# ChaoqinRobotics/LINS---LiDAR-inertial-SLAM

Measured on AMD Instinct MI355X. Metric: ESKF iterations/sec (16x1800 VLP-16, ~2k feat), higher is better.
Workload: dtype f64 state / f32 points

## Files before the change

lins---lidar-inertial-slam_amd/csrc/ieskf_lds_impl.h:

```cpp

#include <hip/hip_runtime.h>

#include "ieskf_binned.h"
#include "ieskf_device.h"
#include "ieskf_grid.h"
#include "icp_math.h"
#include "icp_wave.h"
#include "ieskf_rowsum.h"

#ifndef LINS_PERSIST
#define LINS_PERSIST 0
#endif
#ifndef LINS_PRIO_SHIFT
#define LINS_PRIO_SHIFT 0
#endif
#ifndef LINS_PRIO_LEVEL
#define LINS_PRIO_LEVEL 3
#endif
#ifndef LINS_WALK_CACHE
#define LINS_WALK_CACHE 1
#endif
#ifndef LINS_SPREAD_S
#define LINS_SPREAD_S 5
#define LINS_SPREAD_C 3
#endif

namespace lins {
namespace LINS_LDS_NS {

struct OutRec {
  double residual_norm, update_norm;
  int iters, converged, diverged, m_surf, m_corner, pad[3];
};

struct KernelArgs {
  DevParams prm;
  const ScanDesc* descs;
  const int* order;
  const GridTables* tabs;
  const double* state_in;
  const double* cov_in;
  const double* lin_in;
  double* state_out;
  double* a6_out;
  double* cov_out;
  OutRec* out;
  lins_pose_record* poses;
  double* sums_out;
  int* counts_out;
  long long* prof_buf;
  double* relay_hdr;
  int* relay_lane;
  int* queue;
  int* relay_err;
  unsigned* walk_cache;
  int run_gen;
  int iter_arg, scan_id_base, relay_n, relay_at, relay_cuts, relay_gen;
  int relay_cap;
  int relay_items;
  int relay_spins;
};
typedef const KernelArgs __attribute__((address_space(4))) * ColdArgs;
__device__ __forceinline__ ColdArgs cold_args() {
  auto p = __builtin_amdgcn_kernarg_segment_ptr();
  asm volatile("" : "+s"(p));
  return (ColdArgs)p;
}

constexpr int kMaxLWaves = LINS_LDS_WAVES;
#ifndef LINS_LDS_BATCH_BLOCK
#define LINS_LDS_BATCH_BLOCK 512
#endif
constexpr int kBatchBlock = LINS_LDS_BATCH_BLOCK;
constexpr int kNpCap = LINS_LDS_CAP;
constexpr int kNpMax = LINS_LDS_NMAX;
constexpr bool kHybrid = kNpMax > kNpCap;
constexpr int kScanBatch = LINS_LDS_SCANBATCH;
static_assert(kNpMax >= kNpCap && kNpMax <= kGridNpMax, "positions are u16, indices u16; the index kernel's cap");

typedef unsigned v4u __attribute__((ext_vector_type(4)));
struct LdsStore {
  float4 pt[kNpCap];
  GridTables gt;
  double P[324];
  double trig[kSincCosTab];
  IterConst ic;
  double filt[19];
  double sums[28];
  double partial[kMaxLWaves * 28 > kIcpWorkspace ? kMaxLWaves * 28 : kIcpWorkspace];
  double aug[3][42];
  double res_prev, res_last, upd_norm;
  int scan_tmp[kMaxLWaves + 4];
  int m_surf, m_corner, iter, conv, div, pad;
  long long prof_acc[16];
#ifdef LINS_PROF_TAIL
  long long prof_tail[2];
#endif
#ifdef LINS_PROF2
  int prof2[64];
  int prof3[32];
#endif
  int dbg[4];
};
static_assert(sizeof(LdsStore) <= LINS_LDS_BYTES, "LDS budget of one workgroup");

__shared__ LdsStore g_lds;

struct LCloud {
  const unsigned short* cell_end;
  const int* ring_start;
  const float2* el_ang;
  int naz, stride, base, n;
  const float4* gs;
  int n_lds;
};

__device__ __forceinline__ void pt_xyz(const LdsStore& L, const LCloud& c, int p, float& x, float& y, float& z) {
  if (!kHybrid || p < c.n_lds) {
    const float4 v = L.pt[p];
    x = v.x, y = v.y, z = v.z;
  } else {
    const float4 g = c.gs[p];
    x = g.x, y = g.y, z = g.z;
  }
}
__device__ __forceinline__ int pt_idx(const LdsStore& L, const LCloud& c, int p) {
  if (!kHybrid || p < c.n_lds) return __float_as_int(L.pt[p].w);
  return __float_as_int(c.gs[p].w);
}
__device__ __forceinline__ float pt_sqdist(const LdsStore& L, const LCloud& c, int p, float sx, float sy, float sz) {
  float x, y, z;
  pt_xyz(L, c, p, x, y, z);
  return sqdist3(x, y, z, sx, sy, sz);
}

struct QueryPolar {
  float rho, qn3, el, inv_unused;
  int a0_surf_or_corner;
};

struct Best {
  unsigned long long k;
  int pos, ring;
  unsigned long long k2;
  int pos2, ring2;
  float omin;
  __device__ __forceinline__ float d() const { return __uint_as_float((unsigned)(k >> 32)); }
  __device__ __forceinline__ int key() const { return (int)(unsigned)k; }
};
__device__ __forceinline__ Best best_init(float thr) {
  return Best{(unsigned long long)__float_as_uint(thr) << 32, -1, -1, 0x7F800000FFFFFFFFull, -1, -1, INFINITY};
}
__device__ __forceinline__ unsigned long long pack_key(float d, int key) {
  return ((unsigned long long)__float_as_uint(d) << 32) | (unsigned)key;
}
__device__ __forceinline__ void insert_key(Best& b, unsigned long long k, int pos, int ring) {
  if (k < b.k) {
    if (b.pos2 >= 0) b.omin = fminf(b.omin, __uint_as_float((unsigned)(b.k2 >> 32)));
    b.k2 = b.k, b.pos2 = b.pos, b.ring2 = b.ring;
    b.k = k, b.pos = pos, b.ring = ring;
  } else if (k > b.k) {
    if (k < b.k2) {
      if (b.pos2 >= 0) b.omin = fminf(b.omin, __uint_as_float((unsigned)(b.k2 >> 32)));
      b.k2 = k, b.pos2 = pos, b.ring2 = ring;
    } else if (k > b.k2) {
      b.omin = fminf(b.omin, __uint_as_float((unsigned)(k >> 32)));
    }
  }
}
__device__ __forceinline__ void consider(Best& b, float d, int key, int pos, int ring) {
  insert_key(b, pack_key(d, key), pos, ring);
}
__device__ __forceinline__ void consider_scan(Best& b, bool ok, float d, int key, int pos, int ring) {
  const bool cand = ok && d <= __uint_as_float((unsigned)(b.k2 >> 32));
  b.omin = (ok && !cand) ? fminf(b.omin, d) : b.omin;
  if (cand) insert_key(b, pack_key(d, key), pos, ring);
}
__device__ __forceinline__ void merge_from_lane(Best& b, int src_lane) {
  unsigned lo = __shfl((unsigned)b.k, src_lane), hi = __shfl((unsigned)(b.k >> 32), src_lane);
  unsigned lo2 = __shfl((unsigned)b.k2, src_lane), hi2 = __shfl((unsigned)(b.k2 >> 32), src_lane);
  int pos = __shfl(b.pos, src_lane), ring = __shfl(b.ring, src_lane);
  int pos2 = __shfl(b.pos2, src_lane), ring2 = __shfl(b.ring2, src_lane);
  float om = __shfl(b.omin, src_lane);
  b.omin = fminf(b.omin, om);
  if (pos >= 0) insert_key(b, ((unsigned long long)hi << 32) | lo, pos, ring);
  if (pos2 >= 0) insert_key(b, ((unsigned long long)hi2 << 32) | lo2, pos2, ring2);
}

template <int LANES>
__device__ __forceinline__ void merge_query_lanes(Best& b, int lane_base, int role, int ln) {
  if (LANES == 3) {
    merge_from_lane(b, lane_base + (role + 1) % 3);
    merge_from_lane(b, lane_base + (role + 2) % 3);
  } else if (LANES != 1) {
    const int n = LANES ? LANES : ln;
#pragma unroll 1
    for (int m = 1; m < n; m <<= 1) merge_from_lane(b, lane_base + (role ^ m));
  }
}

__device__ __forceinline__ float bound_sqrtf(float x) { return __builtin_amdgcn_sqrtf(x); }

__device__ __forceinline__ float bound_divf(float x, float y) { return x * __frcp_rn(y) * (1.f + 3e-7f); }

__device__ __forceinline__ float cert_lb(const Best& b, float thr, float margin) {
  return fminf(bound_sqrtf(b.omin), bound_sqrtf(b.pos >= 0 ? b.d() : thr) + margin);
}
__device__ __forceinline__ bool certified(float d_now, float lb, float drift) {
  return bound_sqrtf(d_now) * (1.f + 4e-6f) + 2e-6f < (lb - drift * (1.f + 4e-6f)) * (1.f - 4e-6f);
}


#ifndef LINS_GLOB_BATCH
#define LINS_GLOB_BATCH 1
#endif
constexpr int kGlobBatch = LINS_GLOB_BATCH;
struct Spans {
  int s0, e0, s1, e1, spans;
  __device__ __forceinline__ int count() const { return (e0 - s0) + (e1 - s1); }
};
__device__ __forceinline__ Spans spans_of(const LCloud& c, int r, int lo, int hi) {
  int s0 = 0, e0 = 0, s1 = 0, e1 = 0, spans = 1;
  if (lo <= hi) {
    const int naz = c.naz, row = r * naz;
    int len = hi - lo;
    if (len >= naz - 1) lo = 0, len = naz - 1;
    lo &= naz - 1;
    hi = lo + len;
    const int c0 = row + lo, c1 = row + (hi < naz ? hi : naz - 1);
    s0 = c0 ? (int)c.cell_end[c0 - 1] : c.base;
    e0 = (int)c.cell_end[c1];
    if (hi >= naz) {
      spans = 2;
      s1 = row ? (int)c.cell_end[row - 1] : c.base;
      e1 = (int)c.cell_end[row + hi - naz];
    }
  }
  return Spans{s0, e0, s1, e1, spans};
}
template <class F>
__device__ __forceinline__ void scan_spans(const LdsStore& L, const LCloud& c, const Spans& w, F f) {
#pragma unroll 1
  for (int k = 0; k < w.spans; ++k) {
    const int s = k ? w.s1 : w.s0, e = k ? w.e1 : w.e0;
    const int el = kHybrid ? (e < c.n_lds ? e : c.n_lds) : e;
#pragma unroll 1
// ... 324 lines not shown
  NnOut r{bb.pos, bb.ring, bb.pos2, bb.ring2, cert_lb(bb, thr, margin)};
  if (ln > 1) {
    const int src = (cm.rank * ln) & 63;
    r.pos = __shfl(r.pos, src), r.ring = __shfl(r.ring, src);
    r.pos2 = __shfl(r.pos2, src), r.ring2 = __shfl(r.ring2, src), r.lb = __shfl(r.lb, src);
  }
  return r;
}
__device__ __forceinline__ WalkOut coop_walk(const LdsStore& L, const LCloud& c, bool is_surf, int nq, const CoopMap& cm, int coop_cap,
                                             bool need_walk, int lane, float sx, float sy, float sz, const QueryPolar& qp, int j1, int rho1,
                                             int w2, int w3, bool nn_changed, float thr, float margin, bool skip) {
  const int ln = coop_lanes(cm.n, coop_cap);
  const int wrole = lane & (ln - 1), wbase = lane - wrole, item = lane / ln;
  bool valid = need_walk;
  float isx = sx, isy = sy, isz = sz;
  QueryPolar iq = qp;
  int i_j1 = j1, i_rho1 = rho1, i_w2 = w2, i_w3 = w3, i_chk = nn_changed;
  if (ln > 1) {
    valid = item < cm.n;
    const int owner = __shfl(cm.owner_map, valid ? item : 0);
    isx = __shfl(sx, owner), isy = __shfl(sy, owner), isz = __shfl(sz, owner);
    iq.rho = __shfl(qp.rho, owner), iq.qn3 = __shfl(qp.qn3, owner), iq.el = __shfl(qp.el, owner);
    iq.a0_surf_or_corner = __shfl(qp.a0_surf_or_corner, owner);
    i_j1 = __shfl(j1, owner), i_rho1 = __shfl(rho1, owner);
    i_w2 = __shfl(w2, owner), i_w3 = __shfl(w3, owner), i_chk = __shfl((int)nn_changed, owner);
  }
  Best c2 = best_init(thr), c3 = c2;
  if (valid && !skip)
    walk_lds<0>(L, c, is_surf, nq, thr, i_j1, i_rho1, isx, isy, isz, iq, margin, ln, wrole, wbase, i_w2, i_w3, i_chk != 0, c2, c3);
  WalkOut r{c2.pos, c2.pos2, c3.pos, c3.pos2, cert_lb(c2, thr, margin), cert_lb(c3, thr, margin)};
  if (ln > 1) {
    const int src = (cm.rank * ln) & 63;
    r.r2 = __shfl(r.r2, src), r.r2b = __shfl(r.r2b, src), r.r3 = __shfl(r.r3, src), r.r3b = __shfl(r.r3b, src);
    r.lb2 = __shfl(r.lb2, src), r.lb3 = __shfl(r.lb3, src);
  }
  return r;
}
constexpr int kRelayLanes = 512;
constexpr int kRelayRegionInts = 4 * kRelayLanes * 4;
constexpr int kRelayLaneInts = kRelayRegionInts;
#ifdef LINS_LDS_LEAN
#include "ieskf_lds_lean.h"
constexpr bool kLeanBuild = true;
#else
constexpr bool kLeanBuild = false;
#endif
__device__ __forceinline__ LCloud make_cloud(const LdsStore& L, bool is_surf, const float4* gs, int n_corner_t, int n_surf_t, int n_lds) {
  return is_surf ? LCloud{L.gt.cell_end + kCellsCorner, L.gt.ring_start[0], &L.gt.el_ang[0][0], kAzSurf, 1, n_corner_t, n_surf_t, gs, n_lds}
                 : LCloud{L.gt.cell_end, L.gt.ring_start[1], &L.gt.el_ang[1][0], kAzCorner, kAzSurf / kAzCorner, 0, n_corner_t, gs, n_lds};
}
template <int BLOCK>
#ifndef LINS_GRID_INLINE
#define LINS_GRID_INLINE 1
#endif
#if LINS_GRID_INLINE
__device__ __forceinline__
#else
__device__ __noinline__
#endif
    void
    load_lds_grid(const GridTables* __restrict__ tab, const float4* __restrict__ gs, int n_lds, int tid) {
  LdsStore& L = g_lds;
  constexpr int kTabPer = (kGridTableWords + BLOCK - 1) / BLOCK, kPtPer = (kNpCap + BLOCK - 1) / BLOCK;
  constexpr int kChunk = kPtPer < 12 ? kPtPer : 12;
  const uint4* src = reinterpret_cast<const uint4*>(tab);
  uint4* dst = reinterpret_cast<uint4*>(&L.gt);
  uint4 tw[kTabPer];
#pragma unroll
  for (int u = 0; u < kTabPer; ++u) tw[u] = src[min(tid + u * BLOCK, kGridTableWords - 1)];
  if (n_lds > 0) {
#pragma unroll
    for (int k0 = 0; k0 < kPtPer; k0 += kChunk) {
      float4 pbuf[kChunk];
#pragma unroll
      for (int u = 0; u < kChunk; ++u) pbuf[u] = gs[min(tid + (k0 + u) * BLOCK, n_lds - 1)];
#pragma unroll
      for (int u = 0; u < kChunk; ++u) L.pt[min(tid + (k0 + u) * BLOCK, n_lds - 1)] = pbuf[u];
    }
  }
#pragma unroll
  for (int u = 0; u < kTabPer; ++u) dst[min(tid + u * BLOCK, kGridTableWords - 1)] = tw[u];
  __syncthreads();
}

#include "ieskf_lds_tail.h"

__device__ __forceinline__ void relay_st(int* p, int v) { __hip_atomic_store(p, v, __ATOMIC_RELAXED, __HIP_MEMORY_SCOPE_AGENT); }
__device__ __forceinline__ int relay_ld(const int* p) { return __hip_atomic_load(p, __ATOMIC_RELAXED, __HIP_MEMORY_SCOPE_AGENT); }
__device__ __forceinline__ void relay_st(double* p, double v) {
  __hip_atomic_store(reinterpret_cast<long long*>(p), __double_as_longlong(v), __ATOMIC_RELAXED, __HIP_MEMORY_SCOPE_AGENT);
}
__device__ __forceinline__ double relay_ld(const double* p) {
  return __longlong_as_double(__hip_atomic_load(reinterpret_cast<const long long*>(p), __ATOMIC_RELAXED, __HIP_MEMORY_SCOPE_AGENT));
}
__device__ __forceinline__ int relay_add(int* p, int v) { return __hip_atomic_fetch_add(p, v, __ATOMIC_RELAXED, __HIP_MEMORY_SCOPE_AGENT); }

#ifndef LINS_RELAY_RELEASE
#define LINS_RELAY_RELEASE 1
#endif
__device__ __forceinline__ void relay_raise(int* p, int v) {
  __hip_atomic_fetch_max(p, v, LINS_RELAY_RELEASE ? __ATOMIC_RELEASE : __ATOMIC_RELAXED, __HIP_MEMORY_SCOPE_AGENT);
}
__device__ __forceinline__ int relay_ld_acq(const int* p) {
  return __hip_atomic_load(p, LINS_RELAY_RELEASE ? __ATOMIC_ACQUIRE : __ATOMIC_RELAXED, __HIP_MEMORY_SCOPE_AGENT);
}

constexpr int kQHead = 0, kQExited = 32, kQFlags = 64;


template <int BLOCK, int LANES, bool PASS_ONLY, bool PROF, bool ICP, bool KNOBS>
__device__ __forceinline__ bool ieskf_lds_update(const KernelArgs ka, const float4* __restrict__ arena, const float4* __restrict__ sorted,
                                                 int4* __restrict__ idx_store, lins_corr* __restrict__ dump, const int scan, const int part) {
  const bool cont = part > 0;
  const DevParams prm = ka.prm;
  const int relay_n = ka.relay_n, relay_at = ka.relay_at;
  const int pad = KNOBS ? prm.pad : 0;
  constexpr bool prof = PROF;
  constexpr int kLBlock = BLOCK, kQPerWave = 64 / LANES, kQPerRound = (BLOCK / 64) * kQPerWave;
  static_assert(BLOCK >= 256 && BLOCK / 64 <= kMaxLWaves, "block shape");
  LdsStore& L = g_lds;
  if (prof && threadIdx.x < 16) g_lds.prof_acc[threadIdx.x] = 0;
#ifdef LINS_PROF2
  if (prof && threadIdx.x < 64) g_lds.prof2[threadIdx.x] = 0;
  if (prof && threadIdx.x < 32) g_lds.prof3[threadIdx.x] = 0;
#define PROF2_ADD(ph, dt)                                                                   \
  do {                                                                                      \
    if (prof && lane == 0 && iter >= LINS_PROF2 && wave < 8) g_lds.prof2[wave * 8 + (ph)] += (int)(dt); \
  } while (0)
#else
#define PROF2_ADD(ph, dt) \
  do {                    \
    (void)sizeof(dt);     \
  } while (0)
#endif
  const long long t_begin = prof ? clock64() : 0, t_wall_begin = prof ? wall_clock64() : 0;
  const int tid = threadIdx.x, lane = tid & 63, wave = __builtin_amdgcn_readfirstlane(tid >> 6);
  constexpr bool kLean = kLeanBuild && LANES == 1 && !PASS_ONLY && !ICP;
  constexpr bool kRelay = kLean && BLOCK == kBatchBlock;
  const ScanDesc sd = ka.descs[scan];
  const int total = sd.n_surf_q + sd.n_corner_q;
  const float4* const gs = sorted + sd.off_surf_t;
  const int n_all_t = sd.n_surf_t + sd.n_corner_t, n_lds = n_all_t < kNpCap ? n_all_t : kNpCap;

  for (int k = tid; k < 324; k += kLBlock) L.P[k] = (PASS_ONLY || ICP) ? 0.0 : ka.cov_in[(size_t)scan * 324 + k];
  if (tid < 19) {
    double v = ka.state_in[(size_t)scan * 19 + tid];
    L.filt[tid] = v;
    L.ic.lin[tid] = PASS_ONLY ? ka.lin_in[(size_t)scan * 19 + tid] : v;
  }
  if (tid < 28) L.sums[tid] = 0;
  if (tid == 64) lins_sinc_cos_table(L.trig);
  if (tid == 0) {
    L.res_prev = 1e6, L.res_last = 0, L.upd_norm = 0;
    L.iter = PASS_ONLY ? ka.iter_arg : 0, L.conv = 0, L.div = 0, L.m_surf = 0, L.m_corner = 0;
    L.dbg[0] = L.dbg[1] = L.dbg[2] = L.dbg[3] = 0;
  }
  __syncthreads();
  if (tid < 64 && !(kRelay && cont)) {
    IterConst ic;
    double filt[19];
    for (int k = 0; k < 19; ++k) ic.lin[k] = L.ic.lin[k], filt[k] = L.filt[k];
    make_iter_const_tail(filt, ic);
    if (tid == 0) {
      L.ic.phi = ic.phi, L.ic.Rt = ic.Rt, L.ic.Gt = ic.Gt;
      for (int k = 0; k < 18; ++k) L.ic.d[k] = ic.d[k];
    }
  }
  load_lds_grid<BLOCK>(ka.tabs + scan, gs, n_lds, tid);
  if (prof && tid == 0) L.prof_acc[0] = clock64() - t_begin;

  const LCloud cs{L.gt.cell_end + kCellsCorner, L.gt.ring_start[0], &L.gt.el_ang[0][0], kAzSurf, 1, sd.n_corner_t, sd.n_surf_t,
                  gs, n_lds};
  const LCloud cc{L.gt.cell_end, L.gt.ring_start[1], &L.gt.el_ang[1][0], kAzCorner, kAzSurf / kAzCorner, 0, sd.n_corner_t,
                  gs, n_lds};
  const int role = lane % LANES, lane_base = lane - role, q_in_wave = lane / LANES;
  const bool lane_used = lane < kQPerWave * LANES;
  struct WrLay {
    int n_wr, k;
    bool kind_s;
    int slot;
    bool active;
  };
  constexpr int kWaves = BLOCK / 64, kSpreadSurf = LINS_SPREAD_S > 0 && BLOCK == kBatchBlock ? LINS_SPREAD_S : (kWaves * 5 + 4) / 8;
  constexpr int kWs = kSpreadSurf;
  constexpr int kWc = LINS_SPREAD_C > 0 && BLOCK == kBatchBlock ? LINS_SPREAD_C : kWaves - kWs;
#ifndef LINS_SPREAD_WS
#define LINS_SPREAD_WS 30, 24, 20, 14, 12
#endif
#ifndef LINS_SPREAD_WC
#define LINS_SPREAD_WC 1, 1, 1
#endif
  constexpr int kWtS[] = {LINS_SPREAD_WS, 1, 1, 1, 1, 1, 1, 1, 1, 1, 1, 1, 1, 1, 1, 1, 1}, kWtC[] = {LINS_SPREAD_WC, 1, 1, 1, 1, 1, 1, 1, 1, 1, 1, 1, 1, 1, 1, 1, 1};
  constexpr int kSpreadMax = 16;
  static_assert(LANES != 1 || kWaves <= kSpreadMax + 1, "spread layout: weights for every wave");
  constexpr bool kWeighted = BLOCK == kBatchBlock && LINS_SPREAD_S > 0;
  auto share_start = [&](const int* wt, int nw, int n, int j) {
    int tot = 0, cum = 0;
#pragma unroll
    for (int k = 0; k < kSpreadMax; ++k) tot += k < nw ? (kWeighted ? wt[k] : 1) : 0, cum += k < j ? (kWeighted ? wt[k] : 1) : 0;
    return j >= nw ? n : (n * cum) / tot;
  };
  bool fits = kWs < kWaves;
#pragma unroll
  for (int k = 0; k < kSpreadMax; ++k) {
    if (k < kWs) fits = fits && share_start(kWtS, kWs, sd.n_surf_q, k + 1) - share_start(kWtS, kWs, sd.n_surf_q, k) <= 64;
    if (k < kWc) fits = fits && share_start(kWtC, kWc, sd.n_corner_q, k + 1) - share_start(kWtC, kWc, sd.n_corner_q, k) <= 64;
  }
  const bool spread_ok = fits;
  auto wr_layout = [&](int rnd) {
    WrLay y;
    y.k = rnd * kWaves + wave;
    if (spread_ok) {
#ifdef LINS_SPREAD_ROLES
      constexpr int kRole[] = {LINS_SPREAD_ROLES, 8, 9, 10, 11, 12, 13, 14, 15, 16};
      const int role_k = (kWeighted && y.k < kWs + kWc && y.k < 8) ? kRole[y.k] : y.k;
#else
      const int role_k = y.k;
#endif
      y.n_wr = kWs + kWc, y.kind_s = role_k < kWs;
      const int j = y.kind_s ? role_k : role_k - kWs, nw = y.kind_s ? kWs : kWc, n = y.kind_s ? sd.n_surf_q : sd.n_corner_q;
      const int q0 = share_start(y.kind_s ? kWtS : kWtC, nw, n, j), q1 = share_start(y.kind_s ? kWtS : kWtC, nw, n, j + 1);
      y.slot = (y.kind_s ? 0 : sd.n_surf_q) + q0 + lane, y.active = y.k < y.n_wr && lane < q1 - q0;
    } else {
      const int nws = (sd.n_surf_q + 63) >> 6;
      y.n_wr = nws + ((sd.n_corner_q + 63) >> 6), y.kind_s = y.k < nws;
      const int q0 = y.kind_s ? y.k * 64 : (y.k - nws) * 64;
      const int left = (y.kind_s ? sd.n_surf_q : sd.n_corner_q) - q0;
      y.slot = (y.kind_s ? 0 : sd.n_surf_q) + q0 + lane, y.active = y.k < y.n_wr && lane < (left < 64 ? left : 64);
    }
    return y;
  };

  int a1 = -1, b1c = -1, ra1 = -1, rb1 = -1;
  int a2 = -1, b2c = -1, a3 = -1, b3c = -1;
  int sel1 = -1;
  float lb1 = 0.f, lb2 = 0.f, lb3 = 0.f, certA[3] = {0.f, 0.f, 0.f}, certB[3] = {0.f, 0.f, 0.f};
  bool have_cert = false;
  bool searched = false;
  constexpr int kRelayHdr = 64;
  static_assert(sizeof(IterConst) == 58 * sizeof(double), "relay header layout");
  static_assert(kGridNpMax < 32768, "grid positions travel as signed 16-bit words");
  if (kRelay && cont) {
    const double* h = ka.relay_hdr + (size_t)scan * kRelayHdr;
    if (tid < 58) reinterpret_cast<double*>(&L.ic)[tid] = relay_ld(h + tid);
    if (tid == 64) L.res_prev = relay_ld(h + 58), L.res_last = relay_ld(h + 59), L.upd_norm = relay_ld(h + 60);
    if (tid == 65) {
      const int* hi = reinterpret_cast<const int*>(h + 61);
      L.iter = relay_ld(hi), L.dbg[0] = relay_ld(hi + 1), L.dbg[1] = relay_ld(hi + 2), L.dbg[2] = relay_ld(hi + 3), L.dbg[3] = relay_ld(hi + 4);
    }
    searched = true;
    __syncthreads();
  }
  bool relay_out = false;
  const int cut_at = (kRelay && relay_n > 0) ? relay_next_cut(L.iter, relay_at, ka.relay_cuts) : 0x7FFFFFFF;
#ifdef LINS_PROF2
  int dbg_nn = 0, dbg_walk = 0, dbg_walk_mask = 0, dbg_slot = -1;
#endif

  for (;;) {
    const int iter = L.iter;
    if (!PASS_ONLY && (iter >= prm.num_iter || L.conv || L.div)) break;
    if (kRelay && iter >= cut_at) {
      relay_out = true;
      break;
    }
    __syncthreads();
    if (tid == 0) L.m_surf = 0, L.m_corner = 0;

    const bool do_search = PASS_ONLY || (iter % prm.icp_freq) == 0;
    double acc = 0;
    int ms = 0, mc = 0;
    long long t0 = prof ? clock64() : 0, t1 = t0, t2 = t0, t3 = t0;
    int surf_waves = (sd.n_surf_q + kQPerWave - 1) / kQPerWave;
    const bool aligned = surf_waves * kQPerWave + sd.n_corner_q <= kQPerRound;
    const int n_wr = LANES == 1 ? wr_layout(0).n_wr : 0;
    const int span = LANES == 1 ? ((n_wr + kWaves - 1) / kWaves) * kQPerRound
                                : (aligned ? surf_waves * kQPerWave + sd.n_corner_q : total);
    int4 held = make_int4(0, 0, 0, -1);
    int part_k = wave;
    for (int base = 0; base < span; base += kQPerRound) {
      const int vslot = base + wave * kQPerWave + q_in_wave;
      int slot = vslot;
      bool active = lane_used && vslot < span;
      bool kind_s = true;
      int wr_k = 0;
      if (LANES == 1) {
        const WrLay y = wr_layout(base / kQPerRound);
        wr_k = y.k, kind_s = y.kind_s, slot = y.slot, active = y.active;
        if (base == 0) part_k = wave;
      } else if (aligned) {
        if (wave < surf_waves)
          active = active && vslot < sd.n_surf_q;
        else
          slot = vslot - surf_waves * kQPerWave + sd.n_surf_q;
      }
      double row[7] = {0, 0, 0, 0, 0, 0, 0};
      if (span > kQPerRound) {
        a1 = b1c = ra1 = rb1 = a2 = b2c = a3 = b3c = sel1 = -1, have_cert = false;
        lb1 = lb2 = lb3 = 0.f;
      }
      if constexpr (kLean) {
#ifdef LINS_LDS_LEAN
#include "ieskf_lds_lean_body.inc"
#endif
      } else if constexpr (LANES == 1) {
        const bool is_surf = kind_s;
        const int qi = is_surf ? slot : slot - sd.n_surf_q;
        const LCloud& c = is_surf ? cs : cc;
        const float thr = prm.nearest_f;
        const bool single_round = span <= kQPerRound;
        const bool warm_iter = single_round && searched;
        const float margin = warm_iter ? prm.margin_warm : prm.margin_cold;
        const bool verify = (pad & 8) != 0;
        const int coop_cap = warm_iter ? kCoopMaxLanes : LINS_COOP_COLD;
        const unsigned long long kNone = ~0ull;
        float4 q = make_float4(0.f, 0.f, 0.f, 0.f);
        V3 phi = L.ic.phi;
        QueryOut o;
        o.accepted = 0;
        o.c[0] = o.c[1] = o.c[2] = o.c[3] = 0.f;
        o.sel[0] = o.sel[1] = o.sel[2] = 0.f;
        QueryPolar qp = {0.f, 0.f, 0.f, 0.f, 0};
        bool qp_ready = false;
        int p1 = -1, p2 = -1, p3 = -1;
        long long s0 = prof ? clock64() : 0, s1 = s0, s2 = s0;
        if (active) {
          if (pad & 0x400000)
            q = make_float4(1.f + lane, 2.f, 0.5f, 3.25f);
          else
            q = arena[(is_surf ? sd.off_surf_q : sd.off_corner_q) + qi];
          V3 t{L.ic.lin[0], L.ic.lin[1], L.ic.lin[2]};
          if (pad & 0x100000)
            o.sel[0] = q.x, o.sel[1] = q.y, o.sel[2] = q.z;
          else
            transform_to_start(prm, phi, t, q, o.sel[0], o.sel[1], o.sel[2], g_lds.trig);
        }
        if (prof) {
          s1 = clock64();
#ifndef LINS_PROF_WAVES
          if (tid == 0) L.prof_acc[6] += s1 - s0;
#endif
          PROF2_ADD(0, s1 - s0);
        }
        auto dist_to = [&](int pos) { return pt_sqdist(L, c, pos, o.sel[0], o.sel[1], o.sel[2]); };
        auto drift_from = [&](const float* cp) {
          float ex = o.sel[0] - cp[0], ey = o.sel[1] - cp[1], ez = o.sel[2] - cp[2];
          return bound_sqrtf(ex * ex + ey * ey + ez * ez);
        };
        if (do_search) {
          if (!single_round) a1 = b1c = a2 = b2c = a3 = b3c = sel1 = -1;
          bool need_nn = false, said = false, flip = false;
          int pred = -1;
          if (active && (pad & 0x80000) && warm_iter) {
            pred = a1, said = true;
          } else if (active) {
            const float da = a1 >= 0 ? dist_to(a1) : INFINITY, db = b1c >= 0 ? dist_to(b1c) : INFINITY;
            bool ok = warm_iter && !(pad & 16) && certified(fminf(fminf(da, db), thr), lb1, drift_from(certA));
            const unsigned long long ka = da < thr ? pack_key(da, pt_idx(L, c, a1)) : kNone;
            const unsigned long long kb = db < thr ? pack_key(db, pt_idx(L, c, b1c)) : kNone;
            flip = kb < ka;
            pred = (flip ? kb : ka) == kNone ? -1 : (flip ? b1c : a1);
            said = ok;
            if (verify) ok = false;
            need_nn = !ok;
          }
          {
            const CoopMap cm = coop_map(need_nn, lane);
#ifdef LINS_PROF2
            if (prof && lane == 0 && iter >= LINS_PROF2 && cm.n) g_lds.prof3[wave * 4 + 0] += 1, g_lds.prof3[wave * 4 + 2] += cm.n;
#endif
            int r_pos = -1, r_ring = -1, r_pos2 = -1, r_ring2 = -1;
            float r_lb = 0.f;
            if (cm.n) {
              if (!(pad & 0x200000)) qp = polar_of(o.sel[0], o.sel[1], o.sel[2], c.naz), qp_ready = true;
              const NnOut r = coop_nn(L, c, cm, coop_cap, need_nn, lane, o.sel[0], o.sel[1], o.sel[2], qp, ring_of(q.w), a1, ra1, thr, margin, (pad & 2) != 0);
              r_pos = r.pos, r_ring = r.ring, r_pos2 = r.pos2, r_ring2 = r.ring2, r_lb = r.lb;
            }
            if (need_nn) {
              p1 = r_pos;
              if (said && p1 != pred) atomicAdd(&L.dbg[0], 1);
              a1 = r_pos, ra1 = r_ring, b1c = r_pos2, rb1 = r_ring2;
              lb1 = r_lb;
              certA[0] = o.sel[0], certA[1] = o.sel[1], certA[2] = o.sel[2];
            } else if (active) {
              p1 = pred;
              if (flip) {
                const int tp = a1, tr = ra1;
                a1 = b1c, ra1 = rb1, b1c = tp, rb1 = tr;
              }
              atomicAdd(&L.dbg[1], 1);
            }
          }
          const bool nn_changed = p1 != sel1;
          bool set_ok = !nn_changed;
          if (LINS_WALK_CACHE && !PASS_ONLY && warm_iter && nn_changed && active && ka.walk_cache && !(pad & 0x800000)) {
            const auto rs = __builtin_amdgcn_make_buffer_rsrc(ka.walk_cache + (size_t)sd.slot_base * 8, 0, total * 32, 0x00020000);
            const unsigned gen16 = (unsigned)ka.run_gen << 16;
            const v4u e0 = __builtin_amdgcn_raw_buffer_load_b128(rs, slot * 32, 0, 16);
            const v4u e1 = __builtin_amdgcn_raw_buffer_load_b128(rs, slot * 32 + 16, 0, 16);
            if (sel1 >= 0) {
              __builtin_amdgcn_raw_buffer_store_b128(v4u{gen16 | (unsigned)sel1, ((unsigned)a2 & 0xFFFFu) | ((unsigned)b2c << 16),
                                                         ((unsigned)a3 & 0xFFFFu) | ((unsigned)b3c << 16), __float_as_uint(lb2)},
                                                     rs, slot * 32, 0, 16);
              __builtin_amdgcn_raw_buffer_store_b128(v4u{__float_as_uint(lb3), __float_as_uint(certB[0]), __float_as_uint(certB[1]),
                                                         __float_as_uint(certB[2])},
                                                     rs, slot * 32 + 16, 0, 16);
            }
            if (p1 >= 0 && e0.x == (gen16 | (unsigned)p1)) {
              a2 = (int)(short)(e0.y & 0xFFFFu), b2c = (int)e0.y >> 16, a3 = (int)(short)(e0.z & 0xFFFFu), b3c = (int)e0.z >> 16;
              lb2 = __uint_as_float(e0.w), lb3 = __uint_as_float(e1.x);
              certB[0] = __uint_as_float(e1.y), certB[1] = __uint_as_float(e1.z), certB[2] = __uint_as_float(e1.w);
              set_ok = true;
            }
          }
          if (active) sel1 = p1;
          if (prof) {
            s2 = clock64();
#ifndef LINS_PROF_WAVES
            if (tid == 0) L.prof_acc[7] += s2 - s1;
#endif
// ... 169 lines not shown
            const bool said = ok;
            if (verify) ok = false;
            if (!ok) {
              if ((pad & 32) && __ffsll(__ballot(1)) - 1 == lane) atomicAdd(&L.dbg[3], 1 + (iter >= 3 ? 1000 : 0));
              Best bb = best_init(thr);
              if (!(pad & 2))
                bb = nn_lds<LANES>(L, c, o.sel[0], o.sel[1], o.sel[2], qp, thr, margin, ring_of(q.w), LANES, role, lane_base,
                                   a1, ra1);
              p1 = bb.pos;
              if (said && p1 != pred && role == 0) atomicAdd(&L.dbg[0], 1);
              a1 = bb.pos, ra1 = bb.ring, b1c = bb.pos2, rb1 = bb.ring2;
              lb1 = cert_lb(bb, thr, margin);
              certA[0] = o.sel[0], certA[1] = o.sel[1], certA[2] = o.sel[2];
            } else {
              p1 = pred;
              if (flip) {
                const int tp = a1, tr = ra1;
                a1 = b1c, ra1 = rb1, b1c = tp, rb1 = tr;
              }
              if (role == 0) atomicAdd(&L.dbg[1], 1);
            }
          }
          const bool nn_changed = p1 != sel1;
          sel1 = p1;
          if (prof) {
            s2 = clock64();
#ifndef LINS_PROF_WAVES
            if (tid == 0) L.prof_acc[7] += s2 - s1;
#endif
          }
          if (p1 >= 0) {
            const int j1 = pt_idx(L, c, p1), rho1 = ra1;
            bool need_walk = nn_changed || !have_cert;
            int pred2 = -1, pred3 = -1;
            bool flip2 = false, flip3 = false, said23 = false;
            if (!need_walk) {
              const WalkCtx w = make_walk_ctx(c, is_surf ? sd.n_surf_q : sd.n_corner_q, j1, rho1);
              const float dB = drift_from(certB);
              auto judge = [&](int pa, int pb, float lb, int& pred, bool& flip) {
                const float da = pa >= 0 ? dist_to(pa) : INFINITY, db = pb >= 0 ? dist_to(pb) : INFINITY;
                int rka = 0, rkb = 0;
                if (pa >= 0) walk_rank(w, pt_idx(L, c, pa), rka);
                if (pb >= 0) walk_rank(w, pt_idx(L, c, pb), rkb);
                const unsigned long long ka = da < thr ? pack_key(da, rka) : kNone;
                const unsigned long long kb = db < thr ? pack_key(db, rkb) : kNone;
                flip = kb < ka;
                pred = (flip ? kb : ka) == kNone ? -1 : (flip ? pb : pa);
                return certified(fminf(fminf(da, db), thr), lb, dB);
              };
              bool ok23 = judge(a2, b2c, lb2, pred2, flip2);
              if (is_surf) ok23 = judge(a3, b3c, lb3, pred3, flip3) && ok23;
              said23 = ok23;
              need_walk = !ok23 || verify;
            }
            if (need_walk) {
              if ((pad & 32) && __ffsll(__ballot(1)) - 1 == lane) atomicAdd(&L.dbg[0], 1 + (iter >= 3 ? 1000 : 0));
              Best c2 = best_init(thr), c3 = c2;
              if (!(pad & 1))
                walk_lds<LANES>(L, c, is_surf, is_surf ? sd.n_surf_q : sd.n_corner_q, thr, j1, rho1, o.sel[0], o.sel[1],
                                o.sel[2], qp, margin, LANES, role, lane_base, a2, a3, nn_changed, c2, c3);
              if (said23 && (c2.pos != pred2 || (is_surf && c3.pos != pred3)) && role == 0) atomicAdd(&L.dbg[0], 1);
              p2 = c2.pos, p3 = c3.pos;
              a2 = c2.pos, b2c = c2.pos2, a3 = c3.pos, b3c = c3.pos2;
              lb2 = cert_lb(c2, thr, margin), lb3 = cert_lb(c3, thr, margin);
              certB[0] = o.sel[0], certB[1] = o.sel[1], certB[2] = o.sel[2];
            } else {
              p2 = pred2, p3 = pred3;
              if (flip2) {
                const int tp = a2;
                a2 = b2c, b2c = tp;
              }
              if (flip3) {
                const int tp = a3;
                a3 = b3c, b3c = tp;
              }
              if (role == 0) atomicAdd(&L.dbg[2], 1);
            }
          }
          have_cert = single_round;
#ifndef LINS_PROF_WAVES
          if (prof && tid == 0) L.prof_acc[8] += clock64() - s2;
#endif
          if (prm.icp_freq > 1 && role == 0) {
            if (ICP && !is_surf)
              held = make_int4(p1, p2, p3, sd.slot_base + slot);
            else
              idx_store[sd.slot_base + slot] = make_int4(p1, p2, p3, 0);
          }
        } else {
          int4 s = idx_store[sd.slot_base + slot];
          p1 = s.x, p2 = s.y, p3 = s.z;
        }
        long long s3 = prof ? clock64() : 0;
        asm volatile("" ::: "memory");
        if (role == 0) {
          auto pt4 = [&](int pos) {
            float4 v = make_float4(0.f, 0.f, 0.f, 0.f);
            pt_xyz(L, c, pos, v.x, v.y, v.z);
            return v;
          };
          if (is_surf) {
            if (p2 >= 0 && p3 >= 0) surf_row(prm, iter, o.sel[0], o.sel[1], o.sel[2], pt4(p1), pt4(p2), pt4(p3), o);
          } else if (p2 >= 0) {
            corner_row(prm, iter, o.sel[0], o.sel[1], o.sel[2], pt4(p1), pt4(p2), o);
          }
          if (o.accepted) {
            if (ICP) {
              const IcpRow ir = icp_row_dev(prm.inv_period, phi.x, phi.y, phi.z, q.x, q.y, q.z, q.w, o.c[0], o.c[1], o.c[2], o.c[3]);
#pragma unroll
              for (int k = 0; k < 7; ++k) row[k] = ir.v[k];
            } else {
              V3 cv{(double)o.c[0], (double)o.c[1], (double)o.c[2]};
              V3 u = cross(V3{(double)q.x, (double)q.y, (double)q.z}, mvec(L.ic.Rt, cv));
              V3 a = mvec(L.ic.Gt, u);
              row[0] = cv.x, row[1] = cv.y, row[2] = cv.z, row[3] = a.x, row[4] = a.y, row[5] = a.z;
              row[6] = prm.lidar_scale * (double)o.c[3];
            }
            if (is_surf)
              ++ms;
            else
              ++mc;
          }
          if (PASS_ONLY && dump) {
            lins_corr r;
            r.ind1 = p1 >= 0 ? pt_idx(L, c, p1) : -1;
            r.ind2 = p2 >= 0 ? pt_idx(L, c, p2) : -1;
            r.ind3 = (is_surf && p3 >= 0) ? pt_idx(L, c, p3) : -1;
            r.accepted = o.accepted;
            for (int k = 0; k < 4; ++k) r.coeff[k] = o.c[k];
            r.sel[0] = o.sel[0], r.sel[1] = o.sel[1], r.sel[2] = o.sel[2], r.sel[3] = q.w;
            dump[sd.slot_base + slot] = r;
          }
        }
#ifndef LINS_PROF_WAVES
        if (prof && tid == 0) L.prof_acc[9] += clock64() - s3;
#endif
      }
      if (prof) t1 = clock64();
#ifdef LINS_PROF_WAVES
      if (prof && lane == 0 && iter >= LINS_PROF_WAVES) L.prof_acc[6 + wave] += t1 - t0;
#endif
      if (!(pad & 0x40000)) {
        const long long r0 = prof ? clock64() : 0;
        const double red = wave_reduce_rows(row, lane);
        if (prof) PROF2_ADD(4, clock64() - r0);
        acc += red;
      }
    }
    if (do_search) searched = true;
    {
      const int sidx28 = reduce_sum_index(lane);
      if (sidx28 >= 0) L.partial[part_k * 28 + sidx28] = acc;
    }
    if (ms) atomicAdd(&L.m_surf, ms);
    if (mc) atomicAdd(&L.m_corner, mc);
    const long long b0 = prof ? clock64() : 0;
    __syncthreads();
    const long long b1 = prof ? clock64() : 0;
    PROF2_ADD(5, b1 - b0);
    if (tid < 28) {
      double sacc = 0;
#pragma unroll
      for (int g = 0; g < BLOCK / 64; ++g) sacc += L.partial[g * 28 + tid];
      L.sums[tid] = sacc;
    }
    __syncthreads();
    if (prof) t2 = clock64();
    PROF2_ADD(6, t2 - b1);
    if (PASS_ONLY && (pad & 4) && !L.conv) {
      __syncthreads();
      if (tid == 0) L.conv = 1;
      continue;
    }
    if (PASS_ONLY) {
      if (ka.sums_out && tid < 28) ka.sums_out[(size_t)scan * 28 + tid] = L.sums[tid];
      if (ka.counts_out && tid == 0) ka.counts_out[scan * 2] = L.m_surf, ka.counts_out[scan * 2 + 1] = L.m_corner;
      return true;
    }

    if (ICP && held.w >= 0 && L.m_surf >= 10) idx_store[held.w] = make_int4(held.x, held.y, held.z, 0);
    if (ICP) {
      if (tid < 64) icp_solve_and_update(tid, iter);
      __syncthreads();
    } else
      t3 = solve_and_update(prm.r2, prm.fixed_iters, pad, tid, iter, prof);
    if (prof) {
      long long t4 = clock64();
      PROF2_ADD(7, t4 - t2);
      if (tid == 0) {
        L.prof_acc[1] += t1 - t0, L.prof_acc[2] += t2 - t1, L.prof_acc[3] += t3 - t2, L.prof_acc[4] += t4 - t3;
#ifndef LINS_PROF_WAVES
        if (iter < 3) L.prof_acc[10 + iter] = t4 - t0;
#endif
      }
    }
  }
  const ColdArgs kp = cold_args();
#define KP(f) kp->f
#ifdef LINS_PROF2
  if (prof && dbg_slot >= 0) idx_store[dbg_slot] = make_int4(dbg_nn, dbg_walk, dbg_walk_mask, ra1 | (a3 >= 0 ? 0x100 : 0));
#endif
  if (prof && tid == 0) {
    long long* prof_out = KP(prof_buf);
    L.prof_acc[5] = clock64() - t_begin;
#ifndef LINS_PROF_WAVES
    L.prof_acc[13] = (long long)(unsigned)__builtin_amdgcn_s_getreg((4 << 0) | (0 << 6) | (31 << 11)) |
                     ((long long)(unsigned)__builtin_amdgcn_s_getreg((20 << 0) | (0 << 6) | (31 << 11)) << 32);
#endif
    L.prof_acc[14] = t_wall_begin, L.prof_acc[15] = wall_clock64();
    for (int k = 0; k < 16; ++k) prof_out[(size_t)scan * 16 + k] = L.prof_acc[k];
#ifdef LINS_PROF2
    int* ext = reinterpret_cast<int*>(prof_out + (size_t)gridDim.x * 16) + (size_t)scan * 64;
    for (int k = 0; k < 64; ++k) ext[k] = (k & 7) == 4 ? (L.prof3[(k >> 3) * 4 + 1] | (L.prof3[(k >> 3) * 4 + 3] << 12) | (L.prof3[(k >> 3) * 4 + 0] << 20) | (L.prof3[(k >> 3) * 4 + 2] << 26)) : L.prof2[k];
#endif
  }

  if (kRelay && relay_out) {
    double* h = KP(relay_hdr) + (size_t)scan * kRelayHdr;
    if (tid < 58) relay_st(h + tid, reinterpret_cast<const double*>(&L.ic)[tid]);
    if (tid == 64) relay_st(h + 58, L.res_prev), relay_st(h + 59, L.res_last), relay_st(h + 60, L.upd_norm);
    if (tid == 65) {
      int* hi = reinterpret_cast<int*>(h + 61);
      relay_st(hi, L.iter), relay_st(hi + 1, L.dbg[0]), relay_st(hi + 2, L.dbg[1]), relay_st(hi + 3, L.dbg[2]), relay_st(hi + 4, L.dbg[3]);
    }
    __builtin_amdgcn_fence(__ATOMIC_RELEASE, "workgroup");
    asm volatile("s_waitcnt vmcnt(0)" ::: "memory");
    __syncthreads();
    if (tid == 0) relay_raise(KP(queue) + kQFlags + scan, KP(relay_gen) * 16 + part + 1);
    return false;
  }
  if (kRelay && relay_n > 0 && tid == 0)
    relay_raise(KP(queue) + kQFlags + scan, KP(relay_gen) * 16 + 15);

  const int div = L.div;
  if (ICP) {
    if (tid < 19) KP(state_out)[(size_t)scan * 19 + tid] = (tid < 3 || (tid >= 6 && tid < 10)) ? L.ic.lin[tid] : L.filt[tid];
  } else {
    if (tid < 19) KP(state_out)[(size_t)scan * 19 + tid] = div ? L.filt[tid] : L.ic.lin[tid];
    if (KP(a6_out) && tid < 21) KP(a6_out)[(size_t)scan * 21 + tid] = L.sums[tid];
  }
  if (tid == 0) {
    OutRec r;
    r.residual_norm = L.res_last, r.update_norm = L.upd_norm;
    r.iters = L.iter, r.converged = L.conv, r.diverged = div;
    r.m_surf = L.m_surf, r.m_corner = L.m_corner;
    r.pad[0] = L.dbg[0], r.pad[1] = (pad & 32) ? L.dbg[3] : L.dbg[1], r.pad[2] = L.dbg[2];
    KP(out)[scan] = r;
  }
  if (KP(poses) && tid < 32) {
    lins_pose_record* pr = KP(poses) + scan;
    const double* st = div ? L.filt : L.ic.lin;
    if (tid < 19) pr->state[tid] = st[tid];
    if (tid == 19) pr->residual_norm = L.res_last;
    if (tid == 20) {
      pr->iters = L.iter, pr->converged = L.conv, pr->diverged = div;
      pr->m_surf = L.m_surf, pr->m_corner = L.m_corner, pr->scan_id = KP(scan_id_base) + scan;
      pr->pad[0] = pr->pad[1] = 0;
    }
  }
  if (!ICP && KP(cov_out)) joseph_epilogue<BLOCK>(KP(prm).r2, div, KP(cov_out) + (size_t)scan * 324, tid);
  return true;
}

template <int BLOCK, int LANES, bool PASS_ONLY, bool PROF, bool ICP = false, bool KNOBS = true>
#if defined(LINS_LDS_NUMVGPR)
__global__ __launch_bounds__(BLOCK) __attribute__((amdgpu_num_vgpr(LINS_LDS_NUMVGPR))) void ieskf_lds_kernel(
#elif LINS_LDS_MINW > 1
__global__ __launch_bounds__(BLOCK, (PASS_ONLY || ICP) ? 1 : LINS_LDS_MINW) void ieskf_lds_kernel(
#else
__global__ __launch_bounds__(BLOCK) void ieskf_lds_kernel(
#endif
    const KernelArgs ka, const float4* __restrict__ arena, const float4* __restrict__ sorted, int4* __restrict__ idx_store,
    lins_corr* __restrict__ dump) {
  constexpr bool kQueue = kLeanBuild && BLOCK == kBatchBlock && LANES == 1 && !PASS_ONLY && !ICP;
  const bool queued = kQueue && ka.relay_n > 0;
  int item;
#ifdef LINS_QUEUE_TRACE
  const long long qt0 = wall_clock64();
  long long qt1 = qt0;
#endif
#if LINS_PERSIST
#pragma unroll 1
  for (;;) {
#endif
  if (kQueue && queued) {
    if (threadIdx.x == 0) {
      int* const Q = ka.queue;
      const int ticket = relay_add(Q + kQHead, 1);
#if LINS_PERSIST
      if (ticket >= ka.relay_items) {
        g_lds.scan_tmp[0] = -2;
      } else {
#endif
      int it = ka.order[ticket];
      const int part = it >> 27, scan = it & 0x7FFFFFF;
      g_lds.scan_tmp[1] = ticket - part * ka.relay_n;
      if (part) {
        const int want = ka.relay_gen * 16 + part;
        int f = relay_ld(Q + kQFlags + scan);
        for (int spins = 0; f < want; ++spins) {
          if (spins >= ka.relay_spins) {
            __hip_atomic_fetch_add(ka.relay_err, 1, __ATOMIC_RELAXED, __HIP_MEMORY_SCOPE_SYSTEM);
            break;
          }
          __builtin_amdgcn_s_sleep(32);
          f = relay_ld(Q + kQFlags + scan);
        }
        if (LINS_RELAY_RELEASE && f == want) f = relay_ld_acq(Q + kQFlags + scan);
        if (f != want) it = -1;
      }
      g_lds.scan_tmp[0] = it;
#if LINS_PERSIST
      }
#endif
    }
    __syncthreads();
    item = g_lds.scan_tmp[0];
#if LINS_PRIO_SHIFT > 0
    if (g_lds.scan_tmp[1] < (ka.relay_n >> LINS_PRIO_SHIFT)) __builtin_amdgcn_s_setprio(LINS_PRIO_LEVEL);
#endif
#ifdef LINS_QUEUE_TRACE
    qt1 = wall_clock64();
#endif
    __syncthreads();
  } else {
    item = ka.order ? ka.order[blockIdx.x] : (int)blockIdx.x;
  }
#if LINS_PERSIST
  if (kQueue && queued && item == -2) break;
#endif
  if (item >= 0)
    ieskf_lds_update<BLOCK, LANES, PASS_ONLY, PROF, ICP, KNOBS>(ka, arena, sorted, idx_store, dump, item & 0x7FFFFFF, kQueue ? item >> 27 : 0);
#if LINS_PERSIST
  if (!(kQueue && queued)) break;
  __syncthreads();
  }
#endif
  if (kQueue && queued && threadIdx.x == 0) {
    int* const Q = cold_args()->queue;
#ifdef LINS_QUEUE_TRACE
    {
      long long* tr = reinterpret_cast<long long*>(Q + kQFlags + cold_args()->relay_cap) + 4 * (size_t)blockIdx.x;
      tr[0] = qt0, tr[1] = qt1, tr[2] = wall_clock64(), tr[3] = item;
    }
#endif
    if (relay_add(Q + kQExited, 1) == (int)gridDim.x - 1) relay_st(Q + kQHead, 0), relay_st(Q + kQExited, 0);
  }
}

#undef KP
#undef PROF2_ADD
}
}
```

lins---lidar-inertial-slam_amd/csrc/ieskf_lds_tail.h:

```cpp
#pragma once

__device__ __noinline__ long long solve_wave0(double prm_r2, int prm_fixed_iters, int lane, bool prof) {
  long long t3 = 0;
  LdsStore& L = g_lds;
  double* const stage = &L.aug[0][0];
  int* const stage_flags = reinterpret_cast<int*>(&L.aug[1][0]);
  {
    double v = 0.0;
    if (lane < 42) {
      const int i = lane / 7, j = lane % 7;
      if (j < 6) {
        v = (i == j ? prm_r2 : 0.0);
#pragma unroll
        for (int k = 0; k < 6; ++k) v += sym6(L.sums, i, k) * L.P[sidx(k) * 18 + sidx(j)];
      } else {
        v = L.sums[21 + i];
#pragma unroll
        for (int k = 0; k < 6; ++k) v += sym6(L.sums, i, k) * L.ic.d[sidx(k)];
      }
    }
    double pls[6] = {0, 0, 0, 0, 0, 0}, dl = 0;
    if (lane < 18) {
#pragma unroll
      for (int k = 0; k < 6; ++k) pls[k] = L.P[lane * 18 + sidx(k)];
      dl = L.ic.d[lane];
    }
    double wsol[6];
#ifdef LINS_PROF_TAIL
    if (prof && lane == 0) L.prof_tail[0] = clock64();
#endif
    wave_gj_solve6(v, lane, wsol);
#ifdef LINS_PROF_TAIL
    asm volatile("" ::"v"(wsol[0]) : "memory");
    if (prof && lane == 0) L.prof_tail[1] = clock64();
#endif
    double dxi = 0;
    if (lane < 18) {
      double sacc = 0;
#pragma unroll
      for (int k = 0; k < 6; ++k) sacc += pls[k] * wsol[k];
      dxi = dl - sacc;
    }
    if (prof) t3 = clock64();
    double lin[19];
#pragma unroll
    for (int k = 0; k < 19; ++k) lin[k] = L.ic.lin[k];
    double dth[3] = {0, 0, 0};
    bool has_nan = false;
    double un = 0;
#pragma unroll
    for (int k = 0; k < 18; ++k) {
      const double vk = readlane_f64(dxi, k);
      has_nan = has_nan || isnan(vk);
      un += vk * vk;
      if (k >= 6 && k < 9)
        dth[k - 6] = vk;
      else
        lin[k < 6 ? k : k + 1] += vk;
    }
    un = sqrt(un);
    const double rn = sqrt(L.sums[27]);
    double res_prev = L.res_prev;
    int div = 0, conv = 0;
    if (has_nan) {
      div = 2, un = L.upd_norm;
    } else if (rn > res_prev * 10) {
      div = 1, un = L.upd_norm;
    } else {
      const Q4 qn = qnormalized(qmul(Q4{lin[6], lin[7], lin[8], lin[9]}, axis2quat_fast(V3{dth[0], dth[1], dth[2]})));
      lin[6] = qn.w, lin[7] = qn.x, lin[8] = qn.y, lin[9] = qn.z;
      if (un <= 1e-2 && !prm_fixed_iters) conv = 1;
      res_prev = rn;
    }
    if (lane == 0) {
#pragma unroll
      for (int k = 0; k < 19; ++k) stage[k] = lin[k];
      stage[19] = rn, stage[20] = res_prev, stage[21] = un;
      stage_flags[0] = div, stage_flags[1] = conv;
    }
  }
  return t3;
}
__device__ __noinline__ void next_iter_consts(int wave, int lane) {
  LdsStore& L = g_lds;
  const double* const stage = &L.aug[0][0];
  {
    const Q4 q{stage[6], stage[7], stage[8], stage[9]};
    if (wave == 0) {
      const M3 Rt = mtrans(qmat(q));
      if (lane == 0) {
#pragma unroll
        for (int k = 0; k < 19; ++k) L.ic.lin[k] = stage[k];
        L.ic.Rt = Rt;
      }
    } else if (wave == 1) {
      V3 phi;
      M3 Gt;
      phi_and_Gt(q, phi, Gt);
      if (lane == 0) L.ic.phi = phi, L.ic.Gt = Gt;
    } else {
      const Q4 qf{L.filt[6], L.filt[7], L.filt[8], L.filt[9]};
      const V3 da = quat2axis_fast(qmul(qinverse(q), qf));
      if (lane == 0) {
#pragma unroll
        for (int k = 0; k < 3; ++k) {
          L.ic.d[0 + k] = L.filt[0 + k] - stage[0 + k];
          L.ic.d[3 + k] = L.filt[3 + k] - stage[3 + k];
          L.ic.d[9 + k] = L.filt[10 + k] - stage[10 + k];
          L.ic.d[12 + k] = L.filt[13 + k] - stage[13 + k];
          L.ic.d[15 + k] = L.filt[16 + k] - stage[16 + k];
        }
        L.ic.d[6] = da.x, L.ic.d[7] = da.y, L.ic.d[8] = da.z;
      }
    }
  }
}
__device__ __forceinline__ long long solve_and_update(double prm_r2, int prm_fixed_iters, int prm_pad, int tid, int iter, bool prof) {
  long long t3 = 0;
  LdsStore& L = g_lds;
  const int lane = tid & 63, wave = __builtin_amdgcn_readfirstlane(tid >> 6);
  if (prm_pad & 0x10000) {
    if (tid == 0) L.iter = iter + 1;
    __syncthreads();
    return t3;
  }
  const double* const stage = &L.aug[0][0];
  const int* const stage_flags = reinterpret_cast<const int*>(&L.aug[1][0]);
#ifdef LINS_PROF_TAIL
  const long long a0 = prof ? clock64() : 0;
#endif
  if (wave == 0) t3 = solve_wave0(prm_r2, prm_fixed_iters, lane, prof);
#ifdef LINS_PROF_TAIL
  const long long a1 = prof ? clock64() : 0;
#endif
  __syncthreads();
#ifdef LINS_PROF_TAIL
  const long long a2 = prof ? clock64() : 0;
#endif
  const int div = stage_flags[0];
  if (wave < 3 && !div) next_iter_consts(wave, lane);
#ifdef LINS_PROF_TAIL
  const long long a3 = prof ? clock64() : 0;
#endif
  if (tid == 0) {
    L.res_last = stage[19], L.res_prev = stage[20], L.upd_norm = stage[21];
    L.conv = stage_flags[1], L.div = div;
    L.iter = iter + 1;
  }
  __syncthreads();
#ifdef LINS_PROF_TAIL
  if (prof && tid == 0) {
    const long long a4 = clock64();
    L.prof_acc[6] += L.prof_tail[0] - a0, L.prof_acc[7] += L.prof_tail[1] - L.prof_tail[0], L.prof_acc[8] += a1 - L.prof_tail[1];
    L.prof_acc[9] += a2 - a1, L.prof_acc[10] += a3 - a2, L.prof_acc[11] += a4 - a3;
  }
#endif
  return t3;
}

struct IcpRow {
  double v[7];
};
__device__ __noinline__ IcpRow icp_row_dev(double inv_period, double phx, double phy, double phz, float px, float py, float pz,
                                           float intensity, float c0, float c1, float c2, float c3) {
  IcpRow r;
  const float c[4] = {c0, c1, c2, c3};
  icp_row(inv_period, V3{phx, phy, phz}, px, py, pz, intensity, c, r.v, r.v[6]);
  return r;
}

__device__ __noinline__ void icp_solve_and_update(int lane, int iter) {
  LdsStore& L = g_lds;
  {
    int conv = 0;
    if (L.m_surf >= 10 && L.m_corner >= 5) {
      static_assert(sizeof(L.partial) >= kIcpWorkspace * sizeof(double) && sizeof(L.aug) >= 48 * sizeof(double), "ICP workspace");
      double* const ws = L.partial;
      double *const JTJ = &L.aug[0][0], *const JTb = JTJ + 36;
      if (lane < 36) {
        const int i = lane / 6, j = lane % 6;
        JTJ[lane] = L.sums[i <= j ? tri6(i, j) : tri6(j, i)];
      }
      if (lane < 6) JTb[lane] = L.sums[21 + lane];
      __builtin_amdgcn_fence(__ATOMIC_RELEASE, "wavefront");
      __builtin_amdgcn_wave_barrier();
      __builtin_amdgcn_fence(__ATOMIC_ACQUIRE, "wavefront");
      double x[6];
      wave_icp_gn_solve(JTJ, JTb, iter, lane, x, ws);
      double t[3] = {L.ic.lin[0], L.ic.lin[1], L.ic.lin[2]};
      Q4 q{L.ic.lin[6], L.ic.lin[7], L.ic.lin[8], L.ic.lin[9]};
      conv = icp_apply(x, t, q) ? 1 : 0;
      const V3 phi = quat2axis(q);
      if (lane == 0) {
        L.ic.lin[0] = t[0], L.ic.lin[1] = t[1], L.ic.lin[2] = t[2];
        L.ic.lin[6] = q.w, L.ic.lin[7] = q.x, L.ic.lin[8] = q.y, L.ic.lin[9] = q.z;
        L.ic.phi = phi;
      }
    }
    if (lane == 0) {
      L.conv = conv;
      L.iter = iter + 1;
    }
  }
}

template <int BLOCK>
__device__ __noinline__ void joseph_epilogue(double r2, int diverged, double* __restrict__ out, int tid) {
  LdsStore& L = g_lds;
  const double* P = L.P;
  if (diverged) {
    for (int k = tid; k < 324; k += BLOCK) out[k] = P[k];
    return;
  }
  double* const sc = reinterpret_cast<double*>(L.pt);
  double* const Ninv = sc;
  double* const Y = sc + 36;
  double* const T1 = sc + 72;
  double* const M = sc + 108;
  double* const D = sc + 144;
  double* const E2 = sc + 252;
  double* const O = sc + 360;
  static_assert(sizeof(L.pt) >= (360 + 324) * sizeof(double), "scratch of the Joseph epilogue");
  __syncthreads();
  const int lane = tid & 63, wave = tid >> 6;
  if (wave < 2) {
    double v = 0.0;
    if (lane < 54) {
      const int i = lane / 9, j = lane % 9;
      if (j < 6) {
        v = (i == j ? r2 : 0.0);
#pragma unroll
        for (int k = 0; k < 6; ++k) v += sym6(L.sums, i, k) * P[sidx(k) * 18 + sidx(j)];
      } else {
        v = (i == 3 * wave + (j - 6)) ? 1.0 : 0.0;
      }
    }
    v = wave_gj_solve6x3(v, lane);
    if (lane < 54 && lane % 9 >= 6) Ninv[(lane / 9) * 6 + 3 * wave + (lane % 9 - 6)] = v;
  }
  __syncthreads();
  if (tid < 36) {
    const int i = tid / 6, j = tid % 6;
    double y = 0;
#pragma unroll
    for (int k = 0; k < 6; ++k) y += Ninv[i * 6 + k] * sym6(L.sums, k, j);
    Y[tid] = y;
  }
  __syncthreads();
  if (tid < 36) {
    const int i = tid / 6, j = tid % 6;
    double t = 0;
#pragma unroll
    for (int k = 0; k < 6; ++k) t += Y[i * 6 + k] * P[sidx(k) * 18 + sidx(j)];
    T1[tid] = t;
  }
  __syncthreads();
  if (tid < 36) {
    const int i = tid / 6, j = tid % 6;
    double m = 0, z = 0;
#pragma unroll
    for (int k = 0; k < 6; ++k) m += T1[i * 6 + k] * Y[j * 6 + k], z += Y[i * 6 + k] * Ninv[j * 6 + k];
    M[tid] = (m + r2 * z) - Y[j * 6 + i];
  }
  __syncthreads();
  if (tid < 216) {
    const int e = tid < 108 ? tid : tid - 108, i = e / 6, b = e % 6;
    const double* W = tid < 108 ? M : Y;
    double acc = 0;
#pragma unroll
    for (int a = 0; a < 6; ++a) acc += P[i * 18 + sidx(a)] * W[a * 6 + b];
    (tid < 108 ? D : E2)[e] = acc;
  }
  __syncthreads();
  for (int e = tid; e < 324; e += BLOCK) {
    const int i = e / 18, j = e % 18;
    double acc = P[e];
#pragma unroll
    for (int b = 0; b < 6; ++b) acc += D[i * 6 + b] * P[j * 18 + sidx(b)] - E2[i * 6 + b] * P[sidx(b) * 18 + j];
    O[e] = acc;
  }
  __syncthreads();
  for (int e = tid; e < 324; e += BLOCK) {
    const int i = e / 18, j = e % 18;
    out[e] = 0.5 * (O[i * 18 + j] + O[j * 18 + i]);
  }
}
```

Before: 20.48 million.

## Double-buffer match counters and drop two block barriers per iteration

```diff
diff --git a/lins---lidar-inertial-slam_amd/csrc/ieskf_lds_impl.h b/lins---lidar-inertial-slam_amd/csrc/ieskf_lds_impl.h
--- a/lins---lidar-inertial-slam_amd/csrc/ieskf_lds_impl.h
+++ b/lins---lidar-inertial-slam_amd/csrc/ieskf_lds_impl.h
@@ -91,7 +91,7 @@
   double aug[3][42];
   double res_prev, res_last, upd_norm;
   int scan_tmp[kMaxLWaves + 4];
-  int m_surf, m_corner, iter, conv, div, pad;
+  int m_surf[2], m_corner[2], iter, conv, div, pad;
   long long prof_acc[16];
 #ifdef LINS_PROF_TAIL
   long long prof_tail[2];
@@ -722,7 +722,7 @@
   if (tid == 64) lins_sinc_cos_table(L.trig);
   if (tid == 0) {
     L.res_prev = 1e6, L.res_last = 0, L.upd_norm = 0;
-    L.iter = PASS_ONLY ? ka.iter_arg : 0, L.conv = 0, L.div = 0, L.m_surf = 0, L.m_corner = 0;
+    L.iter = PASS_ONLY ? ka.iter_arg : 0, L.conv = 0, L.div = 0, L.m_surf[0] = L.m_surf[1] = 0, L.m_corner[0] = L.m_corner[1] = 0;
     L.dbg[0] = L.dbg[1] = L.dbg[2] = L.dbg[3] = 0;
   }
   __syncthreads();
@@ -834,8 +834,8 @@
       relay_out = true;
       break;
     }
-    __syncthreads();
-    if (tid == 0) L.m_surf = 0, L.m_corner = 0;
+    const int mpar = iter & 1;
+    if (tid == 0) L.m_surf[mpar ^ 1] = 0, L.m_corner[mpar ^ 1] = 0;
 
     const bool do_search = PASS_ONLY || (iter % prm.icp_freq) == 0;
     double acc = 0;
@@ -1311,33 +1311,38 @@
       const int sidx28 = reduce_sum_index(lane);
       if (sidx28 >= 0) L.partial[part_k * 28 + sidx28] = acc;
     }
-    if (ms) atomicAdd(&L.m_surf, ms);
-    if (mc) atomicAdd(&L.m_corner, mc);
+    if (ms) atomicAdd(&L.m_surf[mpar], ms);
+    if (mc) atomicAdd(&L.m_corner[mpar], mc);
     const long long b0 = prof ? clock64() : 0;
     __syncthreads();
     const long long b1 = prof ? clock64() : 0;
     PROF2_ADD(5, b1 - b0);
-    if (tid < 28) {
-      double sacc = 0;
-#pragma unroll
-      for (int g = 0; g < BLOCK / 64; ++g) sacc += L.partial[g * 28 + tid];
-      L.sums[tid] = sacc;
-    }
-    __syncthreads();
+    if (tid < 64) {
+      if (tid < 28) {
+        double sacc = 0;
+#pragma unroll
+        for (int g = 0; g < BLOCK / 64; ++g) sacc += L.partial[g * 28 + tid];
+        L.sums[tid] = sacc;
+      }
+      __builtin_amdgcn_fence(__ATOMIC_RELEASE, "wavefront");
+      __builtin_amdgcn_wave_barrier();
+      __builtin_amdgcn_fence(__ATOMIC_ACQUIRE, "wavefront");
+    }
     if (prof) t2 = clock64();
     PROF2_ADD(6, t2 - b1);
     if (PASS_ONLY && (pad & 4) && !L.conv) {
       __syncthreads();
-      if (tid == 0) L.conv = 1;
+      if (tid == 0) L.conv = 1, L.m_surf[mpar] = 0, L.m_corner[mpar] = 0;
+      __syncthreads();
       continue;
     }
     if (PASS_ONLY) {
       if (ka.sums_out && tid < 28) ka.sums_out[(size_t)scan * 28 + tid] = L.sums[tid];
-      if (ka.counts_out && tid == 0) ka.counts_out[scan * 2] = L.m_surf, ka.counts_out[scan * 2 + 1] = L.m_corner;
+      if (ka.counts_out && tid == 0) ka.counts_out[scan * 2] = L.m_surf[mpar], ka.counts_out[scan * 2 + 1] = L.m_corner[mpar];
       return true;
     }
 
-    if (ICP && held.w >= 0 && L.m_surf >= 10) idx_store[held.w] = make_int4(held.x, held.y, held.z, 0);
+    if (ICP && held.w >= 0 && L.m_surf[mpar] >= 10) idx_store[held.w] = make_int4(held.x, held.y, held.z, 0);
     if (ICP) {
       if (tid < 64) icp_solve_and_update(tid, iter);
       __syncthreads();
@@ -1392,6 +1397,7 @@
     relay_raise(KP(queue) + kQFlags + scan, KP(relay_gen) * 16 + 15);
 
   const int div = L.div;
+  const int mlast = (L.iter - 1) & 1;
   if (ICP) {
     if (tid < 19) KP(state_out)[(size_t)scan * 19 + tid] = (tid < 3 || (tid >= 6 && tid < 10)) ? L.ic.lin[tid] : L.filt[tid];
   } else {
@@ -1402,7 +1408,7 @@
     OutRec r;
     r.residual_norm = L.res_last, r.update_norm = L.upd_norm;
     r.iters = L.iter, r.converged = L.conv, r.diverged = div;
-    r.m_surf = L.m_surf, r.m_corner = L.m_corner;
+    r.m_surf = L.m_surf[mlast], r.m_corner = L.m_corner[mlast];
     r.pad[0] = L.dbg[0], r.pad[1] = (pad & 32) ? L.dbg[3] : L.dbg[1], r.pad[2] = L.dbg[2];
     KP(out)[scan] = r;
   }
@@ -1413,7 +1419,7 @@
     if (tid == 19) pr->residual_norm = L.res_last;
     if (tid == 20) {
       pr->iters = L.iter, pr->converged = L.conv, pr->diverged = div;
-      pr->m_surf = L.m_surf, pr->m_corner = L.m_corner, pr->scan_id = KP(scan_id_base) + scan;
+      pr->m_surf = L.m_surf[mlast], pr->m_corner = L.m_corner[mlast], pr->scan_id = KP(scan_id_base) + scan;
       pr->pad[0] = pr->pad[1] = 0;
     }
   }
diff --git a/lins---lidar-inertial-slam_amd/csrc/ieskf_lds_tail.h b/lins---lidar-inertial-slam_amd/csrc/ieskf_lds_tail.h
--- a/lins---lidar-inertial-slam_amd/csrc/ieskf_lds_tail.h
+++ b/lins---lidar-inertial-slam_amd/csrc/ieskf_lds_tail.h
@@ -173,7 +173,7 @@
   LdsStore& L = g_lds;
   {
     int conv = 0;
-    if (L.m_surf >= 10 && L.m_corner >= 5) {
+    if (L.m_surf[iter & 1] >= 10 && L.m_corner[iter & 1] >= 5) {
       static_assert(sizeof(L.partial) >= kIcpWorkspace * sizeof(double) && sizeof(L.aug) >= 48 * sizeof(double), "ICP workspace");
       double* const ws = L.partial;
       double *const JTJ = &L.aug[0][0], *const JTb = JTJ + 36;
```

Measured after the change: 20.50 million (median of 4 runs). About the same (+0.1%).
